# SunJiamei/LRP-ImageCaptioning

Hardware: AMD Instinct MI355X
Metric: LRP heatmaps/sec (per predicted token) VGG16+adaptive-attn, 224x224 (higher is better)
Workload: dtype bf16x3; 1 GPU; batch=32 synthetic 224x224 per GPU, VGG16 + adaptive-attention, LRP per-token heat-maps, 10 words/caption, V=10000 (BASELINE configs[1]); parallelism=image-sharded x1, RCCL weight broadcast, reverse_walk_precision=bf16x3, handles_per_gpu=2

## Files before the change

lrp-imagecaptioning_amd/csrc/conv_args.h:

```cpp
#pragma once

namespace lrp {

enum ConvPrec { PREC_FP32 = 0, PREC_BF16X3 = 1, PREC_F16X2 = 2 };

enum ConvEpi {
  EPI_BIAS_RELU = 0,
  EPI_BIAS = 1,
  EPI_MUL = 2,
  EPI_MUL_UP2 = 3,
  EPI_FWD_DUAL = 4,
  EPI_STORE = 5,
  EPI_IMG_STENCIL = 6
};
constexpr int IMG_PATCH = 16, IMG_TILE = 14;
constexpr int ACT_MAX_SLOTS = 64;

constexpr int LDS_STRIDE = 32;

constexpr int HALO_PITCH = 16, HALO_PL = 4;
constexpr int conv_halo_rows(int BM) { return BM == 256 ? 352 : 192; }

}

// ... 17 lines not shown
    lo[q] = (_Float16)(r[q] - (float)hi[q]);
  }
  u32x4* d = reinterpret_cast<u32x4*>(dst);
  d[0] = __builtin_bit_cast(u32x4, hi);
  d[1] = __builtin_bit_cast(u32x4, lo);
}
__device__ __forceinline__ void split8_store(const float* r, float* dst) {
  bf16x8 hi, lo;
#pragma unroll
  for (int q = 0; q < 8; ++q) {
    hi[q] = (__bf16)r[q];
    lo[q] = (__bf16)(r[q] - (float)hi[q]);
  }
  u32x4* d = reinterpret_cast<u32x4*>(dst);
  d[0] = __builtin_bit_cast(u32x4, hi);
  d[1] = __builtin_bit_cast(u32x4, lo);
}
__device__ __forceinline__ void conv_divmod(int x, int d, float inv, int& q, int& r) {
  q = (int)(((float)x + 0.5f) * inv);
  r = x - q * d;
  if (r < 0) { --q; r += d; } else if (r >= d) { ++q; r -= d; }
}

struct TileOrder {
  std::vector<int> sig;
  int H = 0, th = 0, nyh = 0, cols_t = 0, tpt = 0;
  bool identity = true;
  int* dev = nullptr;
  int* pinned = nullptr;
  size_t cap = 0;
  hipEvent_t ev = nullptr;
  TileOrder() = default;
  TileOrder(const TileOrder&) = delete;
  TileOrder& operator=(const TileOrder&) = delete;
  ~TileOrder() {
    if (dev) (void)hipFree(dev);
    if (pinned) (void)hipHostFree(pinned);
    if (ev) (void)hipEventDestroy(ev);
  }
};

struct ConvArgs {
  const float* in;
  const float* wpk;
  const float* wpk_frag;
  int NB, H, W, Cin, CinP;
  int N;
  int taps;
  int M;
  int m_tiles, n_tiles;
  const float* bias;
  float* out;
  float* out2;
  const float* aux;
// ... 19 lines not shown
  const int* row2img_host;
  const float* tok_fac;
  unsigned* tok_max_out;
  const float* in_unscale;
  unsigned* act_max_out;
  float* pairs_out;
  const float* pairs_scale;
  int skip_out;
  int scale_per_img, img_rows, n_imgs;
  const float* up2_src;
  int gate_none;
  const unsigned char* up2_gpos;
  int up2_pairs;
  const float* img_w;
  float* img_part;
  int tpt;
  int epi_generic;
  float* pool_gc;
  unsigned char* pool_pos;
  float* pool_x;
  const float* aux_b;
  float* out_b;
  int ostride;
};

}
#endif
```

lrp-imagecaptioning_amd/csrc/conv_igemm.h:

```cpp
#pragma once
#include <hip/hip_runtime.h>
#include <stdint.h>

#include "conv_args.h"
#include "conv_plan.h"
#include "conv_tile.h"

namespace lrp {

__device__ __attribute__((aligned(16))) float lrp_zero_page[4] = {0.f, 0.f, 0.f, 0.f};


template <int WM, int WN, int TM, int TN, int EPI, int PREC, bool HALO = false, bool BREG = false, int TERMS = 7, int NS = 2,
          bool GMASK = false, bool PW = false, bool DG = false>
__global__ __launch_bounds__(64 * WM * WN, BREG && WM * WN != 8 && TN == 1 ? 3 : NS > 2 ? 2 : conv_min_waves(WM * WN, TM, TN, HALO)) void conv_igemm_kernel(ConvArgs a) {
#if defined(__HIP_DEVICE_COMPILE__)
  using T = ConvKernelTraits<WM, WN, TM, TN, EPI, PREC, HALO, BREG, TERMS, NS, GMASK, PW, DG>;
  __shared__ __attribute__((aligned(16))) float smem[T::SMEM];

  const int nblk = a.m_tiles * a.n_tiles;
  int logical;
  {
    const int bid = blockIdx.x, q = nblk >> 3, r = nblk & 7, xcd = bid & 7, idx = bid >> 3;
    logical = (xcd < r ? xcd * (q + 1) : r * (q + 1) + (xcd - r) * q) + idx;
  }
  const int mt = logical / a.n_tiles, nt = logical - mt * a.n_tiles;
  const int m0 = mt * T::BM, n0 = nt * T::BN;
  int pn = 0, py0 = 0, px0 = 0;
  if constexpr (EPI == EPI_IMG_STENCIL) {
    const int tpi = a.tiles_x * a.tiles_y;
    pn = mt / tpi;
    const int r = mt - pn * tpi, ty = r / a.tiles_x;
    py0 = ty * IMG_TILE;
    px0 = (r - ty * a.tiles_x) * IMG_TILE;
  }
  int Y0 = 0, x0 = 0, img0 = 0;
  if constexpr (HALO) {
    const int mtp = a.tile_map ? a.tile_map[mt] : mt;
    const int tyt = mtp / a.cols_t;
    x0 = (mtp - tyt * a.cols_t) * a.tw;
    if (a.tpt > 0) {
      img0 = tyt / a.tpt;
      Y0 = img0 * a.H + (tyt - img0 * a.tpt) * a.th;
    } else {
      Y0 = tyt * a.th;
      img0 = Y0 / a.H;
    }
  }
  const int yend = HALO ? (a.tpt > 0 && (img0 + 1) * a.H < a.nyh ? (img0 + 1) * a.H : a.nyh) : 0;
  const float inv_tw = HALO ? 1.0f / (float)a.tw : 0.f, inv_H = HALO ? 1.0f / (float)a.H : 0.f;
  const float inv_H1 = HALO ? 1.0f / (float)(a.H + 1) : 0.f;
  int simg0 = 0;
  float us0 = 1.f, us1 = 1.f, ps0 = 1.f, ps1 = 1.f;
  [[maybe_unused]] const float inv_img_rows = EPI == EPI_FWD_DUAL && a.scale_per_img ? 1.0f / (float)a.img_rows : 0.f;
  if constexpr (EPI == EPI_FWD_DUAL) {
    if (a.dual_il) {
      int simg1 = 0;
      if (a.scale_per_img) {
        simg0 = HALO ? img0 : m0 / a.img_rows;
        simg1 = simg0 + 1 < a.n_imgs ? simg0 + 1 : simg0;
      }
      if constexpr (PREC == PREC_F16X2) { us0 = a.in_unscale[simg0]; us1 = a.in_unscale[simg1]; }
      if (a.pairs_out) { ps0 = a.pairs_scale[simg0]; ps1 = a.pairs_scale[simg1]; }
    }
  }

  const int tid = threadIdx.x, lane = tid & 63, wave = tid >> 6;
  const int wm = wave / WN, wn = wave - wm * WN;
  const int HW = a.H * a.W;
  const int K = a.taps * a.CinP;
  const int cpt = a.CinP >> 5;
  const int nk = a.taps * cpt;

  int prow = lane >> 3, pchk = lane & 7;
  const int wave_s = __builtin_amdgcn_readfirstlane(wave);
  typedef __attribute__((address_space(3))) void* lptr_t;
  constexpr int OOB = (int)0x80000000;
  constexpr int RSRC_FLAGS = 0x00020000;
  const __amdgpu_buffer_rsrc_t rsB =
      __builtin_amdgcn_make_buffer_rsrc((void*)(a.wpk + (size_t)n0 * K), 0, T::BN * K * 4, RSRC_FLAGS);
  int bvo[T::BP];
#pragma unroll
  for (int p = 0; p < T::BP; ++p) {
    const int r = (wave_s * T::BP + p) * 8 + prow;
    bvo[p] = (r * K + ((pchk ^ ((r >> 1) & 7)) << 2)) * 4;
  }
  const float* abase = HALO ? a.in + (size_t)(Y0 > 0 ? Y0 - 1 : 0) * a.W * a.Cin
                       : EPI == EPI_IMG_STENCIL ? a.in + (size_t)pn * HW * a.Cin
                            : a.in + ((long)m0 - (a.taps == 1 ? 0 : a.W + 1)) * (long)a.Cin;
  const __amdgpu_buffer_rsrc_t rsA = __builtin_amdgcn_make_buffer_rsrc((void*)abase, 0, 0x7FFFFFFF, RSRC_FLAGS);
  int avo[HALO ? 1 : T::AP];
// ... 143 lines not shown
  [[maybe_unused]] auto pw_store = [&](const PwItem& w, int it, int chunk, int abuf) {
    if (it >= pw_items) return;
    const PwPos r = pw_locate(it, chunk);
#pragma unroll
    for (int dx = 0; dx < 2; ++dx) {
      const int hx = 2 * r.wx + dx - (x0 - 1);
      if (hx < 0 || hx >= HALO_PITCH) continue;
      const unsigned j = (unsigned)((r.dy << 1) | dx);
      u32x4 mh, ml;
#pragma unroll
      for (int d = 0; d < 4; ++d) {
        const unsigned p0 = (w.q[d >> 1] >> (16 * (d & 1))) & 0xFFu, p1 = (w.q[d >> 1] >> (16 * (d & 1) + 8)) & 0xFFu;
        const unsigned m = r.valid ? ((p0 == j ? 0x0000FFFFu : 0u) | (p1 == j ? 0xFFFF0000u : 0u)) : 0u;
        mh[d] = w.hi[d] & m;
        ml[d] = w.lo[d] & m;
      }
      const int row = r.hy * HALO_PITCH + hx;
      const int swzu = ((r.hy * a.tw + hx - 1) >> 1) & 7;
      const int dst = abuf * T::STAGE + row * LDS_STRIDE + (((2 * r.g) ^ swzu) << 2);
      *reinterpret_cast<u32x4*>(smem + dst) = mh;
      *reinterpret_cast<u32x4*>(smem + (dst ^ 4)) = ml;
    }
  };
  [[maybe_unused]] PwItem pwi{};
  if constexpr (T::BREGC) {
    if constexpr (PW) {
      pw_load(pwi, tid, 0); pw_store(pwi, tid, 0, 0);
      if (tid + T::NT < pw_items) { pw_load(pwi, tid + T::NT, 0); pw_store(pwi, tid + T::NT, 0, 0); }
    } else
    for (int p = wave_s; p < halo_np; p += T::NW) fire_halo_piece(prep_halo_piece(p, 0, true), p, 0);
  } else if constexpr (BREG) {
    if (PREC == PREC_BF16X3 && a.up2_src) {
      const int Hp = a.H >> 1, Wp = a.W >> 1;
      const int h0 = Y0 - img0 * a.H;
      const int wy0 = (h0 - 1) >> 1, wx0 = (x0 - 1) >> 1;
      const int nwx = ((x0 + a.tw) >> 1) - wx0 + 1, nwy = ((h0 + a.th) >> 1) - wy0 + 1;
      const int items = nwy * nwx * 8;
      const int ntok = img0 < a.NB ? img0 : a.NB - 1;
      const int img = a.row2img ? a.row2img[ntok] : ntok;
      const float inv_nwx = 1.0f / (float)nwx;
      constexpr int UW = 2;
      typedef unsigned u32x2_ __attribute__((ext_vector_type(2)));
      for (int it0 = tid; it0 < items; it0 += T::NT * UW) {
        f32x4 pv[UW][2];
        u32x2_ qv[UW];
        int wyv[UW], wxv[UW], cgv[UW];
        bool okv[UW];
#pragma unroll
        for (int u = 0; u < UW; ++u) {
          const int item = it0 + u * T::NT;
          const int cg = item & 7, wdx = item >> 3;
          int wr, wc;
          conv_divmod(wdx, nwx, inv_nwx, wr, wc);
          const int wy = wy0 + wr, wx = wx0 + wc;
// ... 395 lines not shown
      if ((kc & (T::FLUSH - 1)) == T::FLUSH - 1) {
#pragma unroll
        for (int i = 0; i < TM; ++i)
#pragma unroll
          for (int j = 0; j < TN; ++j) {
            tot[i][j] += acc[i][j];
#pragma unroll
            for (int r = 0; r < 16; ++r) acc[i][j][r] = 0.f;
          }
      }
    }
    buf = nbuf;
  }
  conv_dma_landed_barrier();
  if constexpr (T::BLOCKED) {
#pragma unroll
    for (int i = 0; i < TM; ++i)
#pragma unroll
      for (int j = 0; j < TN; ++j) acc[i][j] += tot[i][j];
  }

  if constexpr (BREG && EPI == EPI_MUL && PREC == PREC_BF16X3 && TM == 2 && TN == 1 && WM == 2 && WN == 2) {
    if (a.img_part) {
      static_assert(2 * T::STAGE >= 128 * 64, "the C tile (then S_1 as pairs, in place; then T) inside the staging LDS");
      constexpr int TS2 = 57;
      float* Cs = smem;
      const float inv_tw2 = 1.0f / (float)a.tw;
      f32x4 gq[4][2];
#pragma unroll
      for (int k = 0; k < 4; ++k) {
        const int item = tid + k * T::NT, row = item >> 3, g = item & 7;
        int ty, tx;
        conv_divmod(row, a.tw, inv_tw2, ty, tx);
        const int Y = Y0 + ty, w = x0 + tx;
        const f32x4 z4 = {0.f, 0.f, 0.f, 0.f};
        gq[k][0] = gq[k][1] = z4;
        if (row < a.th * a.tw && Y < yend && w < a.W) {
          int n, h;
          conv_divmod(Y, a.H, inv_H, n, h);
          const int img = a.row2img ? a.row2img[n] : n;
          const float* gp = a.aux + ((size_t)img * HW + h * a.W + w) * a.N + g * 8;
          gq[k][0] = *reinterpret_cast<const f32x4*>(gp); gq[k][1] = *reinterpret_cast<const f32x4*>(gp + 4);
        }
      }
      u32x4 wq[2][2][2][2];
      {
        const int h2 = lane >> 5;
#pragma unroll
        for (int cc = 0; cc < 2; ++cc)
#pragma unroll
          for (int st = 0; st < 2; ++st)
#pragma unroll
            for (int hl = 0; hl < 2; ++hl)
#pragma unroll
              for (int j = 0; j < 2; ++j)
                wq[cc][st][hl][j] = *reinterpret_cast<const u32x4*>(a.img_w + (size_t)(j * 32 + (lane & 31)) * 64 + cc * 32 + (4 * st + 2 * h2 + hl) * 4);
      }
#pragma unroll
      for (int i = 0; i < TM; ++i)
#pragma unroll
        for (int r = 0; r < 16; ++r)
          Cs[((wm * TM + i) * 32 + (r & 3) + 8 * (r >> 2) + 4 * (lane >> 5)) * 64 + wn * 32 + (lane & 31)] = acc[i][0][r];
      __syncthreads();
#pragma unroll
      for (int k = 0; k < 4; ++k) {
        const int item = tid + k * T::NT, row = item >> 3, g = item & 7;
        float* rp = Cs + row * 64 + (g >> 2) * 32;
        const f32x4 c0 = *reinterpret_cast<const f32x4*>(rp + (g & 3) * 8), c1 = *reinterpret_cast<const f32x4*>(rp + (g & 3) * 8 + 4);
        float v[8];
#pragma unroll
        for (int e = 0; e < 4; ++e) { v[e] = c0[e] * gq[k][0][e]; v[4 + e] = c1[e] * gq[k][1][e]; }
        bf16x8 hi, lo;
#pragma unroll
        for (int q = 0; q < 8; ++q) {
          hi[q] = (__bf16)v[q];
          lo[q] = (__bf16)(v[q] - (float)hi[q]);
        }
        const int d = ((2 * (g & 3)) ^ ((row >> 1) & 7)) << 2;
        *reinterpret_cast<u32x4*>(rp + d) = __builtin_bit_cast(u32x4, hi);
        *reinterpret_cast<u32x4*>(rp + (d ^ 4)) = __builtin_bit_cast(u32x4, lo);
      }
      __syncthreads();
      f32x16 t2[2];
#pragma unroll
      for (int j = 0; j < 2; ++j)
#pragma unroll
        for (int r = 0; r < 16; ++r) t2[j][r] = 0.f;
      {
        const int a_row = wave * 32 + (lane & 31), swz2 = (lane >> 1) & 7, h2 = lane >> 5;
#pragma unroll
        for (int cc = 0; cc < 2; ++cc)
#pragma unroll
          for (int st = 0; st < 2; ++st) {
            const bf16x8 ah = __builtin_bit_cast(bf16x8, *reinterpret_cast<const u32x4*>(Cs + a_row * 64 + cc * 32 + (((4 * st + 2 * h2) ^ swz2) << 2)));
            const bf16x8 al = __builtin_bit_cast(bf16x8, *reinterpret_cast<const u32x4*>(Cs + a_row * 64 + cc * 32 + (((4 * st + 2 * h2 + 1) ^ swz2) << 2)));
#pragma unroll
            for (int j = 0; j < 2; ++j) {
              const bf16x8 bh = __builtin_bit_cast(bf16x8, wq[cc][st][0][j]), bl = __builtin_bit_cast(bf16x8, wq[cc][st][1][j]);
              t2[j] = __builtin_amdgcn_mfma_f32_32x32x16_bf16(al, bh, t2[j], 0, 0, 0);
              t2[j] = __builtin_amdgcn_mfma_f32_32x32x16_bf16(ah, bl, t2[j], 0, 0, 0);
              t2[j] = __builtin_amdgcn_mfma_f32_32x32x16_bf16(ah, bh, t2[j], 0, 0, 0);
            }
          }
      }
      __syncthreads();
      float* Ts = smem;
#pragma unroll
      for (int r = 0; r < 16; ++r) {
        const int lr = wave * 32 + (r & 3) + 8 * (r >> 2) + 4 * (lane >> 5);
#pragma unroll
        for (int j = 0; j < 2; ++j) {
          const int col = j * 32 + (lane & 31);
          if (col < TS2) Ts[lr * TS2 + col] = t2[j][r];
        }
      }
      __syncthreads();
      const int RW = a.tw + 2, npos = (a.th + 2) * RW;
      const int mtp_ = a.tile_map ? a.tile_map[mt] : mt;
      for (int p = tid; p < npos; p += T::NT) {
        const int ry = p / RW, rx = p - ry * RW, oy = ry - 1, ox = rx - 1;
        float pos[3] = {0.f, 0.f, 0.f}, neg[3] = {0.f, 0.f, 0.f};
#pragma unroll
        for (int tap = 0; tap < 9; ++tap) {
          const int sy = oy - (tap / 3 - 1), sx = ox - (tap % 3 - 1);
          if (sy >= 0 && sy < a.th && sx >= 0 && sx < a.tw && Y0 + sy < yend && x0 + sx < a.W) {
            const float* r = Ts + (sy * a.tw + sx) * TS2 + tap * 6;
            pos[0] += r[0]; pos[1] += r[1]; pos[2] += r[2];
            neg[0] += r[3]; neg[1] += r[4]; neg[2] += r[5];
          }
        }
        float* o = a.img_part + ((size_t)mtp_ * npos + p) * 6;
        o[0] = pos[0]; o[1] = pos[1]; o[2] = pos[2]; o[3] = neg[0]; o[4] = neg[1]; o[5] = neg[2];
      }
      return;
    }
  }

  if constexpr (EPI == EPI_IMG_STENCIL) {
    constexpr int TS = T::BN + 1;
    static_assert(T::BM == IMG_PATCH * IMG_PATCH && T::BN == 64 && T::BM * TS <= 2 * T::STAGE, "patch tile is 256 x 64");
    float* Ts = smem;
#pragma unroll
    for (int i = 0; i < TM; ++i)
#pragma unroll
      for (int r = 0; r < 16; ++r) {
        const int lr = (wm * TM + i) * 32 + (r & 3) + 8 * (r >> 2) + 4 * (lane >> 5);
#pragma unroll
        for (int j = 0; j < TN; ++j) Ts[lr * TS + (wn * TN + j) * 32 + (lane & 31)] = acc[i][j][r];
      }
    __syncthreads();
    for (int o = tid; o < IMG_TILE * IMG_TILE; o += T::NT) {
      const int oy = o / IMG_TILE, ox = o - oy * IMG_TILE;
      const int y = py0 + oy, x = px0 + ox;
      if (y >= a.H || x >= a.W) continue;
      float pos[3] = {0.f, 0.f, 0.f}, neg[3] = {0.f, 0.f, 0.f};
#pragma unroll
      for (int tap = 0; tap < 9; ++tap) {
        const float* r = Ts + ((oy + 2 - tap / 3) * IMG_PATCH + (ox + 2 - tap % 3)) * TS + tap * 6;
        pos[0] += r[0]; pos[1] += r[1]; pos[2] += r[2];
// ... 585 lines not shown
```

lrp-imagecaptioning_amd/csrc/conv_launch.h:

```cpp
#pragma once
#include <string.h>
#include <algorithm>
#include <utility>
#include <vector>

#include "common.h"
#include "conv_igemm.h"
#include "conv_plan.h"

namespace lrp {

inline const int* conv_tile_order(const ConvArgs& a, hipStream_t st) {
  if (!sw().tile_order || !a.order || !a.row2img_host || a.NB < 2 || a.th < 1) return nullptr;
  TileOrder& o = *a.order;
  const int tiles_y = a.tpt > 0 ? a.NB * a.tpt : (a.nyh + a.th - 1) / a.th;
  const bool same = o.H == a.H && o.th == a.th && o.nyh == a.nyh && o.cols_t == a.cols_t && o.tpt == a.tpt && (int)o.sig.size() == a.NB &&
                    memcmp(o.sig.data(), a.row2img_host, (size_t)a.NB * sizeof(int)) == 0;
  if (same) return o.identity ? nullptr : o.dev;
  o.sig.assign(a.row2img_host, a.row2img_host + a.NB);
  o.H = a.H; o.th = a.th; o.nyh = a.nyh; o.cols_t = a.cols_t; o.tpt = a.tpt;
  constexpr int band = 1, strip = 2;
  std::vector<long long> key((size_t)tiles_y);
  for (int ty = 0; ty < tiles_y; ++ty) {
    int Ym = a.tpt > 0 ? (ty / a.tpt) * a.H + (ty % a.tpt) * a.th + a.th / 2 : ty * a.th + a.th / 2;
    if (a.tpt > 0 && Ym > (ty / a.tpt + 1) * a.H - 1) Ym = (ty / a.tpt + 1) * a.H - 1;
    if (Ym > a.nyh - 1) Ym = a.nyh - 1;
    const int t = Ym / a.H, hpos = Ym - t * a.H;
    key[ty] = ((long long)o.sig[t] << 42) | ((long long)(hpos / (a.th * band)) << 21) | (long long)t;
  }
  std::vector<int> rows((size_t)tiles_y);
  for (int i = 0; i < tiles_y; ++i) rows[i] = i;
// ... 19 lines not shown
    if (o.dev) (void)hipFree(o.dev);
    if (o.pinned) (void)hipHostFree(o.pinned);
    o.dev = o.pinned = nullptr;
    o.cap = 0;
    if (hipMalloc((void**)&o.dev, m_tiles * sizeof(int)) != hipSuccess ||
        hipHostMalloc((void**)&o.pinned, m_tiles * sizeof(int), hipHostMallocDefault) != hipSuccess) {
      (void)hipGetLastError();
      o.sig.clear();
      return nullptr;
    }
    o.cap = m_tiles;
  }
  memcpy(o.pinned, map.data(), m_tiles * sizeof(int));
  if (!o.ev) (void)hipEventCreateWithFlags(&o.ev, hipEventDisableTiming);
  if (hipMemcpyAsync(o.dev, o.pinned, m_tiles * sizeof(int), hipMemcpyHostToDevice, st) != hipSuccess) {
    (void)hipGetLastError();
    o.sig.clear();
    return nullptr;
  }
  (void)hipEventRecord(o.ev, st);
  return o.dev;
}

inline ConvAsk conv_ask(int epi, int prec, int terms, bool gmask, const ConvArgs& a) {
  ConvAsk q;
  q.epi = epi; q.prec = prec; q.terms = terms; q.gmask = gmask;
  q.NB = a.NB; q.H = a.H; q.W = a.W; q.N = a.N; q.Cin = a.Cin; q.taps = a.taps;
  q.frag = a.wpk_frag != nullptr; q.join = a.join != nullptr; q.dual_il = a.dual_il != 0; q.split = a.split;
  q.up2_src = a.up2_src != nullptr; q.img_part = a.img_part != nullptr; q.pool_gc = a.pool_gc != nullptr;
  q.dual_mul = a.out_b != nullptr;
  return q;
}
inline void conv_apply_plan(const ConvPlan& p, ConvArgs& a) {
  a.M = p.M; a.m_tiles = p.m_tiles; a.n_tiles = p.n_tiles;
  a.tw = p.tw; a.th = p.th; a.hrows = p.hrows; a.cols_t = p.cols_t; a.nyh = p.nyh; a.tpt = p.tpt;
  a.epi_generic = p.epi_generic;
}

template <int PREC>
inline hipError_t conv_launch_img(ConvArgs a, hipStream_t st) {
  if (!a.ximg || (PREC == PREC_F16X2 && !a.tok_fac)) return hipErrorInvalidValue;
  const ConvPlan p = conv_plan(conv_ask(EPI_IMG_STENCIL, PREC, 7, false, a));
  if (!p.ok) return hipErrorInvalidValue;
  if (a.NB <= 0) return hipSuccess;
  conv_apply_plan(p, a);
  a.tiles_x = (a.W + IMG_TILE - 1) / IMG_TILE;
  a.tiles_y = (a.H + IMG_TILE - 1) / IMG_TILE;
  hipLaunchKernelGGL((conv_igemm_kernel<4, 1, 2, 2, EPI_IMG_STENCIL, PREC>), dim3(a.m_tiles), dim3(p.threads), 0, st, a);
  return hipGetLastError();
}

template <int I, int EPI, int PREC, int TERMS, bool GMASK, bool DG>
inline bool conv_launch_form(const ConvPlan& p, ConvArgs& a, hipStream_t st) {
  constexpr ConvFormTile F = CONV_FORM_TILES[I];
  if constexpr (conv_kernel_exists(F.form, F.BM, F.BN, F.pw, EPI, PREC, TERMS, GMASK, DG)) {
    if (p.form != F.form || p.BM != F.BM || p.BN != F.BN || p.pw != F.pw) return false;
    constexpr ConvKernelShape K = conv_kernel_shape(F.form, F.BM, F.BN, F.pw);
    if (K.HALO && (EPI == EPI_MUL || EPI == EPI_MUL_UP2)) a.tile_map = conv_tile_order(a, st);
    hipLaunchKernelGGL((conv_igemm_kernel<K.WM, K.WN, K.TM, K.TN, EPI, PREC, K.HALO, K.BREG, TERMS, K.NS, GMASK, K.PW, DG>),
                       dim3(p.m_tiles * p.n_tiles), dim3(p.threads), 0, st, a);
    return true;
  }
  return false;
}
template <int EPI, int PREC, int TERMS, bool GMASK, bool DG, int... I>
inline bool conv_launch_forms(const ConvPlan& p, ConvArgs& a, hipStream_t st, std::integer_sequence<int, I...>) {
  return (conv_launch_form<I, EPI, PREC, TERMS, GMASK, DG>(p, a, st) || ...);
}

template <int EPI, int PREC, int TERMS = 7, bool GMASK = false, bool DG = false>
inline hipError_t conv_launch_epi(ConvArgs a, hipStream_t st) {
  static_assert(EPI != EPI_IMG_STENCIL && conv_epi_exists(EPI, PREC, TERMS, GMASK, DG), "conv_plan.h: no kernel has this epilogue in this format");
  constexpr bool MUL = EPI == EPI_MUL || EPI == EPI_MUL_UP2, FWD = EPI == EPI_BIAS || EPI == EPI_BIAS_RELU || EPI == EPI_FWD_DUAL;
  if (DG != (a.out_b != nullptr)) return hipErrorInvalidValue;
  if (DG && (!a.aux || !a.aux_b || !a.out || a.ostride < a.N || (a.ostride & (PREC != PREC_FP32 ? 7 : 3)) || a.out2s || a.gate_none ||
             a.gate_binary || a.relu_out))
    return hipErrorInvalidValue;
  if (GMASK && (a.out2s || a.gate_none)) return hipErrorInvalidValue;
  if (PREC == PREC_F16X2 && MUL && (!a.tok_fac || !a.tok_max_out || a.out_plain)) return hipErrorInvalidValue;
  if (PREC == PREC_F16X2 && FWD && !a.in_unscale) return hipErrorInvalidValue;
// ... 40 lines not shown
```

lrp-imagecaptioning_amd/csrc/conv_plan.h:

```cpp
#pragma once
#include "conv_args.h"
#include "switches.h"

namespace lrp {

struct ConvTile { int BM, BN; };
inline ConvTile conv_pick_tile(int N) {
  if (N > 64) return {128, 128};
  if (N > 32) return {128, 64};
  return {128, 32};
}
inline int conv_npad(int N) { ConvTile t = conv_pick_tile(N); return (N + t.BN - 1) / t.BN * t.BN; }
inline int conv_cinp(int Cin) { return (Cin + 31) / 32 * 32; }

enum ConvForm {
  FORM_PLAIN = 0,
  FORM_SMALL = 1,
  FORM_HALO = 2,
  FORM_BREG = 3,
  FORM_POOL = 4,
  FORM_IMG = 5,
  FORM_BREG8 = 6,
  FORM_BREG4 = 7,
  FORM_BREG4_POOL = 8
// ... 63 lines not shown
struct ConvKernelShape { int WM, WN, TM, TN; bool HALO, BREG; int NS; bool PW; };
constexpr ConvKernelShape conv_kernel_shape(int form, int BM, int BN, bool pw) {
  const bool breg = form == FORM_BREG || form == FORM_BREG8 || form == FORM_BREG4 || form == FORM_BREG4_POOL;
  const bool halo = breg || form == FORM_HALO || form == FORM_POOL;
  const int ns = form == FORM_SMALL ? CONV_SMALL_NS : 2;
  if (form == FORM_IMG) return {4, 1, 2, 2, false, false, 2, false};
  if (BM == 256) return {2, 4, 4, 2, halo, breg, ns, pw};
  if (BM == 64) return {2, 2, 1, 1, halo, breg, ns, pw};
  if (BN == 128) return {2, 2, 2, 2, halo, breg, ns, pw};
  if (BN == 64) return {2, 2, 2, 1, halo, breg, ns, pw};
  return {4, 1, 1, 1, halo, breg, ns, pw};
}
constexpr bool conv_kernel_instantiated(int WM, int WN, int TM, int TN, bool HALO, bool BREG, int NS, bool PW, int epi, int prec, int terms,
                                        bool gmask, bool dual) {
  for (const ConvFormTile& f : CONV_FORM_TILES) {
    const ConvKernelShape k = conv_kernel_shape(f.form, f.BM, f.BN, f.pw);
    if (k.WM == WM && k.WN == WN && k.TM == TM && k.TN == TN && k.HALO == HALO && k.BREG == BREG && k.NS == NS && k.PW == PW &&
        conv_kernel_exists(f.form, f.BM, f.BN, f.pw, epi, prec, terms, gmask, dual))
      return true;
  }
  return false;
}

inline float conv_halo_geom(int BM, int H, int W, bool even, int& tw, int& th, int& hrows) {
  const int avail = conv_halo_rows(BM) / HALO_PITCH;
  const int step = even ? 2 : 1;
  float best = 0.f;
  for (int c = step; c <= HALO_PITCH - 2 && c <= W; c += step) {
    int t = even ? (BM / c) & ~1 : BM / c;
    while (t > 0 && t + 2 + (t - 1 + H - 1) / H > avail) t -= step;
    if (t < step) continue;
    const int cols = (W + c - 1) / c;
    const float u = (float)(t * c) / (float)BM * (float)W / (float)(cols * c);
    if (u > best + 1e-6f) { best = u; tw = c; th = t; hrows = t + 2 + (t - 1 + H - 1) / H; }
  }
  return best;
}

inline bool conv_compact_shape(int N, int Cin, int H, int W) {
  if ((Cin & 7) || (H & 1) || (W & 1)) return false;
  return conv_pick_tile(N).BN == 128  || (N <= 64 && conv_cinp(Cin) <= 64) ;
}

inline unsigned conv_frag_forms(int epi, int prec, int terms, int N, int Cin, int taps, const Switches& s = sw()) {
  if (taps != 9 || N <= 0 || (Cin & 7)) return 0;
  auto has = [&](int form, int BM, int BN) { return conv_kernel_exists(form, BM, BN, false, epi, prec, terms, false, false); };
// ... 105 lines not shown
```

lrp-imagecaptioning_amd/csrc/conv_tile.h:

```cpp
#pragma once
#include <hip/hip_runtime.h>
#include <stdint.h>

#include "conv_args.h"
#include "conv_plan.h"

namespace lrp {

constexpr int conv_min_waves(int NW, int TM, int TN, bool halo = false) { return NW == 8 || halo ? 2 : (TM * TN >= 4 ? 2 : 3); }

template <int WM_, int WN_, int TM_, int TN_, int EPI_, int PREC_, bool HALO_, bool BREG_, int TERMS_, int NS_, bool GMASK_, bool PW_, bool DG_>
struct ConvKernelTraits {
  static constexpr int WM = WM_, WN = WN_, TM = TM_, TN = TN_, EPI = EPI_, PREC = PREC_, TERMS = TERMS_, NS = NS_;
  static constexpr bool HALO = HALO_, BREG = BREG_, GMASK = GMASK_, PW = PW_, DG = DG_;

  static constexpr int NW = WM * WN, NT = 64 * NW;
  static constexpr bool SPLIT = PREC != PREC_FP32;
  static constexpr int BM = WM * TM * 32, BN = WN * TN * 32;
  static constexpr int AP = BM / 8 / NW, BP = BN / 8 / NW;
  static constexpr int HR = conv_halo_rows(BM);
  static constexpr int ABUF = (HALO ? HR : BM) * LDS_STRIDE;
  static constexpr int STAGE = ABUF + (BREG ? 0 : BN) * LDS_STRIDE;
  static constexpr bool BREG8 = BREG && NW == 8;
  static constexpr bool BREG4 = BREG && NW == 4 && TN == 2;
// ... 11 lines not shown
  static constexpr int CSLAB = BREGC ? SMEM : 2 * STAGE;

  static constexpr int NSTEP = SPLIT ? 2 : 4;
  static_assert(!BREG || NSTEP == 2, "weights in registers: split operands");
  static_assert(!BREGC || SMEM >= 2 * STAGE + NW * 8 * LDS_STRIDE, "a spare LDS slot per wave behind the two images");
  static_assert(!BREGC || 6 * NW * 8 >= HR, "six piece slots per wave cover the resident image");
  static constexpr int FLUSH = 8;
  static constexpr bool BLOCKED = PREC == PREC_FP32 || (PREC == PREC_F16X2 && (EPI == EPI_BIAS || EPI == EPI_BIAS_RELU || EPI == EPI_FWD_DUAL));

  static constexpr bool SLABS = EPI != EPI_STORE && EPI != EPI_IMG_STENCIL;
  static constexpr int NH = (BM * BN + CSLAB - 1) / CSLAB;
  static constexpr int RH = BM / NH;
  static_assert(!SLABS || (BM % NH == 0 && RH % (TM * 32) == 0 && RH * BN <= CSLAB), "slab must hold whole wave tiles");
  static constexpr bool SPLIT_OUT = SPLIT && (EPI == EPI_MUL || EPI == EPI_MUL_UP2);
  static constexpr int CW = SPLIT_OUT ? 8 : 4;
  static constexpr int C4 = BN / CW, RPP = NT / C4;
  static constexpr bool TMAX_LDS = PREC == PREC_F16X2 && RH * BN + 16 <= 2 * STAGE;
};

__device__ __forceinline__ void conv_dma_landed_barrier() {
  asm volatile("s_waitcnt vmcnt(0)" ::: "memory");
  __syncthreads();
}
template <class T>
__device__ __forceinline__ void conv_dma_oldest_landed_barrier() {
  if constexpr (T::NS > 2) {
    asm volatile("s_waitcnt vmcnt(%0)" ::"n"((T::NS - 2) * T::DPC) : "memory");
    __syncthreads();
  } else {
    conv_dma_landed_barrier();
  }
}

}
```

lrp-imagecaptioning_amd/csrc/switches.h:

```cpp
#pragma once
#include <cstdlib>

namespace lrp {

struct Switches {
  int conv_halo = 1;
  int conv_breg = 1;
  int conv_breg8 = 1;
  int conv_breg4 = 1;
  int conv_sparse_wreg = 1;
  int conv_small = 1;
  int conv_mid = 1;
  int epi_fast = 1;
  int up2_pw = 1;
  int tile_order = 1;
  int fwd_emit = 1;
  int fwd_il = 1;
  int img_fused = 1;
  int up2_compact = 1;
  int img_fold = 1;
  int pool_fused = 1;
  int sparse_pool = 1;
  void load() {
    *this = Switches();
    auto rd = [](const char* name, int& v) { if (const char* e = getenv(name)) v = atoi(e); };
    rd("LRP_CONV_HALO", conv_halo); rd("LRP_CONV_BREG", conv_breg); rd("LRP_CONV_SMALL", conv_small);
    rd("LRP_CONV_MID", conv_mid); rd("LRP_EPI_FAST", epi_fast); rd("LRP_UP2_PW", up2_pw); rd("LRP_TILE_ORDER", tile_order);
    rd("LRP_FWD_EMIT", fwd_emit); rd("LRP_FWD_IL", fwd_il); rd("LRP_IMG_FUSED", img_fused); rd("LRP_UP2_COMPACT", up2_compact);
    rd("LRP_IMG_FOLD", img_fold); rd("LRP_SPARSE_POOL", sparse_pool); rd("LRP_POOL_FUSED", pool_fused);
    if (const char* e = getenv("LRP_CONV_BREG8")) conv_breg8 = atoi(e);
    if (const char* e = getenv("LRP_CONV_BREG4")) conv_breg4 = atoi(e);
    if (const char* e = getenv("LRP_CONV_SPARSE_WREG")) conv_sparse_wreg = atoi(e);
  }
};
inline Switches& sw() {
  static Switches s = [] { Switches t; t.load(); return t; }();
  return s;
}

}
```

Baseline: 11200 heatmaps/s.

## Process runs of same-image tokens per block in the BREG image-part conv

Adds a run-table path for the BF16x3 EPI_MUL image-part kernel. Each block now loops over several tokens that share an image and tile position, so the block setup, weight registers and gate loads are reused across tokens. The next token's up2 source data is prefetched during the current token's epilogue. A host-built, cached run table sets the grid size, and the run length is chosen so the grid still fills the CUs. The cost is fewer blocks, a serial per-block loop, and extra register pressure and code complexity.

```diff
diff --git a/lrp-imagecaptioning_amd/csrc/conv_args.h b/lrp-imagecaptioning_amd/csrc/conv_args.h
--- a/lrp-imagecaptioning_amd/csrc/conv_args.h
+++ b/lrp-imagecaptioning_amd/csrc/conv_args.h
@@ -63,6 +63,23 @@
   if (r < 0) { --q; r += d; } else if (r >= d) { ++q; r -= d; }
 }
 
+struct RunCache {
+  std::vector<int> sig;
+  int tpt = 0, cols_t = 0, cap = 0;
+  int n_runs = 0, n_toks = 0;
+  int* dev = nullptr;
+  int* pinned = nullptr;
+  size_t size = 0;
+  hipEvent_t ev = nullptr;
+  RunCache() = default;
+  RunCache(const RunCache&) = delete;
+  RunCache& operator=(const RunCache&) = delete;
+  ~RunCache() {
+    if (dev) (void)hipFree(dev);
+    if (pinned) (void)hipHostFree(pinned);
+    if (ev) (void)hipEventDestroy(ev);
+  }
+};
 struct TileOrder {
   std::vector<int> sig;
   int H = 0, th = 0, nyh = 0, cols_t = 0, tpt = 0;
@@ -71,6 +88,7 @@
   int* pinned = nullptr;
   size_t cap = 0;
   hipEvent_t ev = nullptr;
+  RunCache runs;
   TileOrder() = default;
   TileOrder(const TileOrder&) = delete;
   TileOrder& operator=(const TileOrder&) = delete;
@@ -136,6 +154,9 @@
   const float* aux_b;
   float* out_b;
   int ostride;
+  const int* run_tab;
+  const int* run_toks;
+  int n_runs;
 };
 
 }
diff --git a/lrp-imagecaptioning_amd/csrc/conv_igemm.h b/lrp-imagecaptioning_amd/csrc/conv_igemm.h
--- a/lrp-imagecaptioning_amd/csrc/conv_igemm.h
+++ b/lrp-imagecaptioning_amd/csrc/conv_igemm.h
@@ -12,13 +12,14 @@
 
 
 template <int WM, int WN, int TM, int TN, int EPI, int PREC, bool HALO = false, bool BREG = false, int TERMS = 7, int NS = 2,
-          bool GMASK = false, bool PW = false, bool DG = false>
+          bool GMASK = false, bool PW = false, bool DG = false, bool RUN = false>
 __global__ __launch_bounds__(64 * WM * WN, BREG && WM * WN != 8 && TN == 1 ? 3 : NS > 2 ? 2 : conv_min_waves(WM * WN, TM, TN, HALO)) void conv_igemm_kernel(ConvArgs a) {
 #if defined(__HIP_DEVICE_COMPILE__)
   using T = ConvKernelTraits<WM, WN, TM, TN, EPI, PREC, HALO, BREG, TERMS, NS, GMASK, PW, DG>;
+  static_assert(!RUN || conv_run_kernel_exists(WM, WN, TM, TN, HALO, BREG, NS, PW, EPI, PREC, TERMS, GMASK, DG), "no such run instantiation: conv_plan.h");
   __shared__ __attribute__((aligned(16))) float smem[T::SMEM];
 
-  const int nblk = a.m_tiles * a.n_tiles;
+  const int nblk = RUN ? a.n_runs : a.m_tiles * a.n_tiles;
   int logical;
   {
     const int bid = blockIdx.x, q = nblk >> 3, r = nblk & 7, xcd = bid & 7, idx = bid >> 3;
@@ -35,8 +36,15 @@
     px0 = (r - ty * a.tiles_x) * IMG_TILE;
   }
   int Y0 = 0, x0 = 0, img0 = 0;
+  [[maybe_unused]] int run_place = 0, run_n = 1, run_first = 0, run_img = 0, cur_tok = 0, nxt_tok = 0, rk = 0;
   if constexpr (HALO) {
-    const int mtp = a.tile_map ? a.tile_map[mt] : mt;
+    int mtp;
+    if constexpr (RUN) {
+      const int4 rd = reinterpret_cast<const int4*>(a.run_tab)[mt];
+      run_place = rd.x & 0xFFFFFF; run_n = rd.x >> 24; run_first = rd.y; run_img = rd.z; cur_tok = rd.w;
+      mtp = cur_tok * (a.tpt * a.cols_t) + run_place;
+    } else
+    mtp = a.tile_map ? a.tile_map[mt] : mt;
     const int tyt = mtp / a.cols_t;
     x0 = (mtp - tyt * a.cols_t) * a.tw;
     if (a.tpt > 0) {
@@ -65,8 +73,8 @@
     }
   }
 
-  const int tid = threadIdx.x, lane = tid & 63, wave = tid >> 6;
-  const int wm = wave / WN, wn = wave - wm * WN;
+  int tid = threadIdx.x, lane = tid & 63, wave = tid >> 6;
+  int wm = wave / WN, wn = wave - wm * WN;
   const int HW = a.H * a.W;
   const int K = a.taps * a.CinP;
   const int cpt = a.CinP >> 5;
@@ -256,6 +264,85 @@
       *reinterpret_cast<u32x4*>(smem + (dst ^ 4)) = ml;
     }
   };
+  constexpr int UWR = 2;
+  typedef unsigned u32x2r __attribute__((ext_vector_type(2)));
+  struct Up2Geom { int Hp, Wp, h0, wy0, wx0, nwx, items; float inv_nwx; };
+  struct Up2Items { f32x4 pv[UWR][2]; u32x2r qv[UWR]; };
+  [[maybe_unused]] auto up2_geom = [&]() {
+    Up2Geom G;
+    G.Hp = a.H >> 1; G.Wp = a.W >> 1;
+    G.h0 = Y0 - img0 * a.H;
+    G.wy0 = (G.h0 - 1) >> 1; G.wx0 = (x0 - 1) >> 1;
+    G.nwx = ((x0 + a.tw) >> 1) - G.wx0 + 1;
+    const int nwy = ((G.h0 + a.th) >> 1) - G.wy0 + 1;
+    G.items = nwy * G.nwx * 8;
+    G.inv_nwx = 1.0f / (float)G.nwx;
+    return G;
+  };
+  [[maybe_unused]] auto up2_item = [&](const Up2Geom& G, int item, int& cg, int& wy, int& wx) {
+    cg = item & 7;
+    int wr, wc;
+    conv_divmod(item >> 3, G.nwx, G.inv_nwx, wr, wc);
+    wy = G.wy0 + wr; wx = G.wx0 + wc;
+    return item < G.items && wy >= 0 && wy < G.Hp && wx >= 0 && wx < G.Wp && cg * 8 < a.Cin;
+  };
+  [[maybe_unused]] auto up2_load = [&](const Up2Geom& G, int it0, int ntok, int img, Up2Items& w) {
+#pragma unroll
+    for (int u = 0; u < UWR; ++u) {
+      int cg, wy, wx;
+      (void)up2_item(G, it0 + u * T::NT, cg, wy, wx);
+      const int wyc = wy < 0 ? 0 : (wy >= G.Hp ? G.Hp - 1 : wy), wxc = wx < 0 ? 0 : (wx >= G.Wp ? G.Wp - 1 : wx);
+      const int cgc = cg * 8 < a.Cin ? cg : 0;
+      const size_t wo = ((size_t)wyc * G.Wp + wxc) * a.Cin + cgc * 8;
+      const float* pp = a.up2_src + (size_t)ntok * G.Hp * G.Wp * a.Cin + wo;
+      w.pv[u][0] = *reinterpret_cast<const f32x4*>(pp); w.pv[u][1] = *reinterpret_cast<const f32x4*>(pp + 4);
+      w.qv[u] = *reinterpret_cast<const u32x2r*>(a.up2_gpos + (size_t)img * G.Hp * G.Wp * a.Cin + wo);
+    }
+  };
+  [[maybe_unused]] auto up2_build = [&](const Up2Geom& G, int it0, const Up2Items& w) {
+#pragma unroll
+    for (int u = 0; u < UWR; ++u) {
+      if (it0 + u * T::NT >= G.items) continue;
+      int cg, wy, wx;
+      const bool ok = up2_item(G, it0 + u * T::NT, cg, wy, wx);
+      const u32x4 z4u = {0u, 0u, 0u, 0u};
+      const u32x4 hiw = ok ? __builtin_bit_cast(u32x4, w.pv[u][0]) : z4u;
+      const u32x4 low = ok ? __builtin_bit_cast(u32x4, w.pv[u][1]) : z4u;
+#pragma unroll
+      for (int j = 0; j < 4; ++j) {
+        const int hy = 2 * wy + (j >> 1) - (G.h0 - 1), hx = 2 * wx + (j & 1) - (x0 - 1);
+        if (hy < 0 || hy >= a.hrows || hx < 0 || hx >= HALO_PITCH) continue;
+        u32x4 mh, ml;
+#pragma unroll
+        for (int d = 0; d < 4; ++d) {
+          const unsigned p0 = (w.qv[u][d >> 1] >> (16 * (d & 1))) & 0xFFu, p1 = (w.qv[u][d >> 1] >> (16 * (d & 1) + 8)) & 0xFFu;
+          const unsigned m = (p0 == (unsigned)j ? 0x0000FFFFu : 0u) | (p1 == (unsigned)j ? 0xFFFF0000u : 0u);
+          mh[d] = hiw[d] & m;
+          ml[d] = low[d] & m;
+        }
+        const int row = hy * HALO_PITCH + hx;
+        const int swzu = ((hy * a.tw + hx - 1) >> 1) & 7;
+        const int dst = (cg >> 2) * T::STAGE + row * LDS_STRIDE + (((2 * (cg & 3)) ^ swzu) << 2);
+        *reinterpret_cast<u32x4*>(smem + dst) = mh;
+        *reinterpret_cast<u32x4*>(smem + (dst ^ 4)) = ml;
+      }
+    }
+  };
+  [[maybe_unused]] Up2Items up2w;
+  if constexpr (RUN) {
+    up2_load(up2_geom(), tid, cur_tok, run_img, up2w);
+    up2_build(up2_geom(), tid, up2w);
+  }
+  do {
+  if constexpr (RUN) {
+    asm volatile("" : "+v"(tid), "+s"(Y0), "+s"(x0), "+s"(img0));
+    lane = tid & 63; wave = tid >> 6;
+    wm = wave / WN; wn = wave - wm * WN;
+#pragma unroll
+    for (int i = 0; i < TM; ++i)
+#pragma unroll
+      for (int r = 0; r < 16; ++r) acc[i][0][r] = 0.f;
+  }
   [[maybe_unused]] PwItem pwi{};
   if constexpr (T::BREGC) {
     if constexpr (PW) {
@@ -264,6 +351,9 @@
     } else
     for (int p = wave_s; p < halo_np; p += T::NW) fire_halo_piece(prep_halo_piece(p, 0, true), p, 0);
   } else if constexpr (BREG) {
+    if constexpr (RUN) {
+      nxt_tok = rk + 1 < run_n ? a.run_toks[run_first + rk + 1] : cur_tok;
+    } else
     if (PREC == PREC_BF16X3 && a.up2_src) {
       const int Hp = a.H >> 1, Wp = a.W >> 1;
       const int h0 = Y0 - img0 * a.H;
@@ -705,11 +795,29 @@
 
   if constexpr (BREG && EPI == EPI_MUL && PREC == PREC_BF16X3 && TM == 2 && TN == 1 && WM == 2 && WN == 2) {
     if (a.img_part) {
+      auto epi_barrier = [] {
+        if constexpr (RUN) conv_lds_barrier();
+        else __syncthreads();
+      };
       static_assert(2 * T::STAGE >= 128 * 64, "the C tile (then S_1 as pairs, in place; then T) inside the staging LDS");
       constexpr int TS2 = 57;
       float* Cs = smem;
       const float inv_tw2 = 1.0f / (float)a.tw;
       f32x4 gq[4][2];
+      [[maybe_unused]] bool okg[4] = {true, true, true, true};
+      if constexpr (RUN) {
+#pragma unroll
+        for (int k = 0; k < 4; ++k) {
+          const int item = tid + k * T::NT, row = item >> 3, g = item & 7;
+          int ty = (int)(((float)row + 0.5f) * inv_tw2), tx = row - ty * a.tw;
+          const int up = tx < 0 ? -1 : tx >= a.tw ? 1 : 0;
+          ty += up; tx -= up * a.tw;
+          const int h = Y0 - img0 * a.H + ty, w = x0 + tx;
+          okg[k] = row < a.th * a.tw && h < a.H && w < a.W;
+          const float* gp = a.aux + ((size_t)run_img * HW + (okg[k] ? h * a.W + w : (Y0 - img0 * a.H) * a.W + x0)) * a.N + g * 8;
+          gq[k][0] = *reinterpret_cast<const f32x4*>(gp); gq[k][1] = *reinterpret_cast<const f32x4*>(gp + 4);
+        }
+      } else
 #pragma unroll
       for (int k = 0; k < 4; ++k) {
         const int item = tid + k * T::NT, row = item >> 3, g = item & 7;
@@ -744,13 +852,17 @@
 #pragma unroll
         for (int r = 0; r < 16; ++r)
           Cs[((wm * TM + i) * 32 + (r & 3) + 8 * (r >> 2) + 4 * (lane >> 5)) * 64 + wn * 32 + (lane & 31)] = acc[i][0][r];
-      __syncthreads();
+      epi_barrier();
 #pragma unroll
       for (int k = 0; k < 4; ++k) {
         const int item = tid + k * T::NT, row = item >> 3, g = item & 7;
         float* rp = Cs + row * 64 + (g >> 2) * 32;
         const f32x4 c0 = *reinterpret_cast<const f32x4*>(rp + (g & 3) * 8), c1 = *reinterpret_cast<const f32x4*>(rp + (g & 3) * 8 + 4);
         float v[8];
+        if constexpr (RUN) {
+          const f32x4 z4 = {0.f, 0.f, 0.f, 0.f};
+          if (!okg[k]) gq[k][0] = gq[k][1] = z4;
+        }
 #pragma unroll
         for (int e = 0; e < 4; ++e) { v[e] = c0[e] * gq[k][0][e]; v[4 + e] = c1[e] * gq[k][1][e]; }
         bf16x8 hi, lo;
@@ -763,7 +875,7 @@
         *reinterpret_cast<u32x4*>(rp + d) = __builtin_bit_cast(u32x4, hi);
         *reinterpret_cast<u32x4*>(rp + (d ^ 4)) = __builtin_bit_cast(u32x4, lo);
       }
-      __syncthreads();
+      epi_barrier();
       f32x16 t2[2];
 #pragma unroll
       for (int j = 0; j < 2; ++j)
@@ -786,7 +898,11 @@
             }
           }
       }
-      __syncthreads();
+      epi_barrier();
+      if constexpr (RUN) {
+        if (rk + 1 < run_n) up2_load(up2_geom(), tid, nxt_tok, run_img, up2w);
+        else up2w = Up2Items{};
+      }
       float* Ts = smem;
 #pragma unroll
       for (int r = 0; r < 16; ++r) {
@@ -797,9 +913,11 @@
           if (col < TS2) Ts[lr * TS2 + col] = t2[j][r];
         }
       }
-      __syncthreads();
+      epi_barrier();
       const int RW = a.tw + 2, npos = (a.th + 2) * RW;
-      const int mtp_ = a.tile_map ? a.tile_map[mt] : mt;
+      int mtp_;
+      if constexpr (RUN) mtp_ = cur_tok * (a.tpt * a.cols_t) + run_place;
+      else mtp_ = a.tile_map ? a.tile_map[mt] : mt;
       for (int p = tid; p < npos; p += T::NT) {
         const int ry = p / RW, rx = p - ry * RW, oy = ry - 1, ox = rx - 1;
         float pos[3] = {0.f, 0.f, 0.f}, neg[3] = {0.f, 0.f, 0.f};
@@ -815,9 +933,18 @@
         float* o = a.img_part + ((size_t)mtp_ * npos + p) * 6;
         o[0] = pos[0]; o[1] = pos[1]; o[2] = pos[2]; o[3] = neg[0]; o[4] = neg[1]; o[5] = neg[2];
       }
+      if constexpr (RUN) {
+        if (++rk < run_n) {
+          cur_tok = nxt_tok;
+          epi_barrier();
+          up2_build(up2_geom(), tid, up2w);
+          continue;
+        }
+      }
       return;
     }
   }
+  } while (RUN);
 
   if constexpr (EPI == EPI_IMG_STENCIL) {
     constexpr int TS = T::BN + 1;
diff --git a/lrp-imagecaptioning_amd/csrc/conv_launch.h b/lrp-imagecaptioning_amd/csrc/conv_launch.h
--- a/lrp-imagecaptioning_amd/csrc/conv_launch.h
+++ b/lrp-imagecaptioning_amd/csrc/conv_launch.h
@@ -7,6 +7,7 @@
 #include "common.h"
 #include "conv_igemm.h"
 #include "conv_plan.h"
+#include "conv_runs.h"
 
 namespace lrp {
 
@@ -72,6 +73,63 @@
   return o.dev;
 }
 
+inline bool conv_run_table(ConvArgs& a, hipStream_t st) {
+  const Switches& s = sw();
+  if (!s.conv_breg_run || s.conv_breg_run_max == 1 || !a.order || !a.row2img_host || !a.row2img || !a.img_part || !a.up2_src ||
+      a.tpt < 1 || a.NB < 2 || a.n_tiles != 1 || a.CinP > 64)
+    return false;
+  if (((a.th + 1) / 2 + 2) * ((a.tw + 1) / 2 + 2) * 8 > 2 * 256) return false;
+  if ((long long)a.NB * a.tpt * a.cols_t > 0x7FFFFFFFLL) return false;
+  RunCache& c = a.order->runs;
+  const bool same = c.tpt == a.tpt && c.cols_t == a.cols_t && c.cap == s.conv_breg_run_max && (int)c.sig.size() == a.NB &&
+                    memcmp(c.sig.data(), a.row2img_host, (size_t)a.NB * sizeof(int)) == 0;
+  if (!same) {
+    c.sig.assign(a.row2img_host, a.row2img_host + a.NB);
+    c.tpt = a.tpt; c.cols_t = a.cols_t; c.cap = s.conv_breg_run_max;
+    c.n_runs = 0;
+    static const int cus = [] {
+      int dev = 0, n = 0;
+      if (hipGetDevice(&dev) != hipSuccess || hipDeviceGetAttribute(&n, hipDeviceAttributeMultiprocessorCount, dev) != hipSuccess) (void)hipGetLastError();
+      return n > 0 ? n : 256;
+    }();
+    const int cap = conv_run_cap(c.sig.data(), a.NB, a.tpt * a.cols_t, cus, s.conv_breg_run_max);
+    if (cap > 1) {
+      ConvRunTable t;
+      conv_build_runs(c.sig.data(), a.NB, a.tpt, a.cols_t, cap, t);
+      const size_t need = t.runs.size() + t.toks.size();
+      if (c.ev) (void)hipEventSynchronize(c.ev);
+      if (c.size < need) {
+        if (c.dev) (void)hipFree(c.dev);
+        if (c.pinned) (void)hipHostFree(c.pinned);
+        c.dev = c.pinned = nullptr;
+        c.size = 0;
+        if (hipMalloc((void**)&c.dev, need * sizeof(int)) != hipSuccess ||
+            hipHostMalloc((void**)&c.pinned, need * sizeof(int), hipHostMallocDefault) != hipSuccess) {
+          (void)hipGetLastError();
+          c.sig.clear();
+          return false;
+        }
+        c.size = need;
+      }
+      if (t.n_runs() > 0) {
+        memcpy(c.pinned, t.runs.data(), t.runs.size() * sizeof(int));
+        memcpy(c.pinned + t.runs.size(), t.toks.data(), t.toks.size() * sizeof(int));
+        if (!c.ev) (void)hipEventCreateWithFlags(&c.ev, hipEventDisableTiming);
+        if (hipMemcpyAsync(c.dev, c.pinned, need * sizeof(int), hipMemcpyHostToDevice, st) != hipSuccess) {
+          (void)hipGetLastError();
+          c.sig.clear();
+          return false;
+        }
+        (void)hipEventRecord(c.ev, st);
+        c.n_runs = t.n_runs(); c.n_toks = (int)t.toks.size();
+      }
+    }
+  }
+  if (c.n_runs < 1) return false;
+  a.run_tab = c.dev; a.run_toks = c.dev + (size_t)c.n_runs * 4; a.n_runs = c.n_runs;
+  return true;
+}
+
 inline ConvAsk conv_ask(int epi, int prec, int terms, bool gmask, const ConvArgs& a) {
   ConvAsk q;
   q.epi = epi; q.prec = prec; q.terms = terms; q.gmask = gmask;
@@ -106,6 +164,13 @@
   if constexpr (conv_kernel_exists(F.form, F.BM, F.BN, F.pw, EPI, PREC, TERMS, GMASK, DG)) {
     if (p.form != F.form || p.BM != F.BM || p.BN != F.BN || p.pw != F.pw) return false;
     constexpr ConvKernelShape K = conv_kernel_shape(F.form, F.BM, F.BN, F.pw);
+    if constexpr (conv_run_kernel_exists(F.form, F.BM, F.BN, F.pw, EPI, PREC, TERMS, GMASK, DG)) {
+      if (conv_run_table(a, st)) {
+        hipLaunchKernelGGL((conv_igemm_kernel<K.WM, K.WN, K.TM, K.TN, EPI, PREC, K.HALO, K.BREG, TERMS, K.NS, GMASK, K.PW, DG, true>),
+                           dim3(a.n_runs), dim3(p.threads), 0, st, a);
+        return true;
+      }
+    }
     if (K.HALO && (EPI == EPI_MUL || EPI == EPI_MUL_UP2)) a.tile_map = conv_tile_order(a, st);
     hipLaunchKernelGGL((conv_igemm_kernel<K.WM, K.WN, K.TM, K.TN, EPI, PREC, K.HALO, K.BREG, TERMS, K.NS, GMASK, K.PW, DG>),
                        dim3(p.m_tiles * p.n_tiles), dim3(p.threads), 0, st, a);
diff --git a/lrp-imagecaptioning_amd/csrc/conv_plan.h b/lrp-imagecaptioning_amd/csrc/conv_plan.h
--- a/lrp-imagecaptioning_amd/csrc/conv_plan.h
+++ b/lrp-imagecaptioning_amd/csrc/conv_plan.h
@@ -109,6 +109,17 @@
   return false;
 }
 
+constexpr bool conv_run_kernel_exists(int form, int BM, int BN, bool pw, int epi, int prec, int terms, bool gmask, bool dual) {
+  return form == FORM_BREG && BM == 128 && BN == 64 && !pw && epi == EPI_MUL && prec == PREC_BF16X3 && !gmask && !dual &&
+         conv_kernel_exists(form, BM, BN, pw, epi, prec, terms, gmask, dual);
+}
+constexpr bool conv_run_kernel_exists(int WM, int WN, int TM, int TN, bool HALO, bool BREG, int NS, bool PW, int epi, int prec, int terms,
+                                      bool gmask, bool dual) {
+  const ConvKernelShape k = conv_kernel_shape(FORM_BREG, 128, 64, false);
+  return k.WM == WM && k.WN == WN && k.TM == TM && k.TN == TN && k.HALO == HALO && k.BREG == BREG && k.NS == NS && k.PW == PW &&
+         conv_run_kernel_exists(FORM_BREG, 128, 64, false, epi, prec, terms, gmask, dual);
+}
+
 inline float conv_halo_geom(int BM, int H, int W, bool even, int& tw, int& th, int& hrows) {
   const int avail = conv_halo_rows(BM) / HALO_PITCH;
   const int step = even ? 2 : 1;
diff --git a/lrp-imagecaptioning_amd/csrc/conv_runs.h b/lrp-imagecaptioning_amd/csrc/conv_runs.h
--- /dev/null
+++ b/lrp-imagecaptioning_amd/csrc/conv_runs.h
@@ -0,0 +1,66 @@
+#pragma once
+#include <algorithm>
+#include <vector>
+
+namespace lrp {
+
+struct ConvRunTable {
+  std::vector<int> toks;
+  std::vector<int> runs;
+  int n_runs() const { return (int)(runs.size() / 4); }
+};
+constexpr int CONV_RUN_MAX = 127;
+constexpr int CONV_RUN_MAX_PLACES = 1 << 24;
+
+inline long conv_run_count(const int* tok2img, int n_tok, int places, int cap) {
+  std::vector<int> img(tok2img, tok2img + n_tok);
+  std::sort(img.begin(), img.end());
+  long runs = 0;
+  for (int i = 0; i < n_tok;) {
+    int j = i;
+    while (j < n_tok && img[j] == img[i]) ++j;
+    runs += (j - i + cap - 1) / cap;
+    i = j;
+  }
+  return runs * places;
+}
+inline int conv_run_cap(const int* tok2img, int n_tok, int places, int cus, int want) {
+  if (n_tok < 1 || places < 1) return 1;
+  if (want > 0) return want < CONV_RUN_MAX ? want : CONV_RUN_MAX;
+  std::vector<int> img(tok2img, tok2img + n_tok);
+  std::sort(img.begin(), img.end());
+  int longest = 1;
+  for (int i = 0, j = 0; i < n_tok; i = j) {
+    while (j < n_tok && img[j] == img[i]) ++j;
+    longest = std::max(longest, j - i);
+  }
+  int cap = std::min(longest, CONV_RUN_MAX);
+  const long fill = 4L * 3 * cus;
+  while (cap > 1 && conv_run_count(tok2img, n_tok, places, cap) < fill) cap = (cap + 1) / 2;
+  return cap;
+}
+
+inline void conv_build_runs(const int* tok2img, int n_tok, int tpt, int cols_t, int cap, ConvRunTable& t) {
+  t.toks.resize((size_t)(n_tok > 0 ? n_tok : 0));
+  t.runs.clear();
+  if (n_tok < 1 || tpt < 1 || cols_t < 1 || (long)tpt * cols_t > CONV_RUN_MAX_PLACES) return;
+  cap = cap < 1 ? 1 : cap > CONV_RUN_MAX ? CONV_RUN_MAX : cap;
+  for (int i = 0; i < n_tok; ++i) t.toks[i] = i;
+  std::stable_sort(t.toks.begin(), t.toks.end(), [&](int x, int y) { return tok2img[x] < tok2img[y]; });
+  constexpr int strip = 2;
+  for (int i0 = 0; i0 < n_tok;) {
+    int i1 = i0;
+    while (i1 < n_tok && tok2img[t.toks[i1]] == tok2img[t.toks[i0]]) ++i1;
+    for (int c0 = 0; c0 < cols_t; c0 += strip)
+      for (int r = 0; r < tpt; ++r)
+        for (int c = c0; c < c0 + strip && c < cols_t; ++c)
+          for (int f = i0; f < i1; f += cap) {
+            const int cnt = std::min(cap, i1 - f);
+            const int rec[4] = {(r * cols_t + c) | (cnt << 24), f, tok2img[t.toks[i0]], t.toks[f]};
+            t.runs.insert(t.runs.end(), rec, rec + 4);
+          }
+    i0 = i1;
+  }
+}
+
+}
diff --git a/lrp-imagecaptioning_amd/csrc/conv_tile.h b/lrp-imagecaptioning_amd/csrc/conv_tile.h
--- a/lrp-imagecaptioning_amd/csrc/conv_tile.h
+++ b/lrp-imagecaptioning_amd/csrc/conv_tile.h
@@ -57,6 +57,7 @@
   asm volatile("s_waitcnt vmcnt(0)" ::: "memory");
   __syncthreads();
 }
+__device__ __forceinline__ void conv_lds_barrier() { asm volatile("s_waitcnt lgkmcnt(0)\n\ts_barrier" ::: "memory"); }
 template <class T>
 __device__ __forceinline__ void conv_dma_oldest_landed_barrier() {
   if constexpr (T::NS > 2) {
diff --git a/lrp-imagecaptioning_amd/csrc/switches.h b/lrp-imagecaptioning_amd/csrc/switches.h
--- a/lrp-imagecaptioning_amd/csrc/switches.h
+++ b/lrp-imagecaptioning_amd/csrc/switches.h
@@ -21,6 +21,8 @@
   int img_fold = 1;
   int pool_fused = 1;
   int sparse_pool = 1;
+  int conv_breg_run = 1;
+  int conv_breg_run_max = 0;
   void load() {
     *this = Switches();
     auto rd = [](const char* name, int& v) { if (const char* e = getenv(name)) v = atoi(e); };
@@ -31,6 +33,8 @@
     if (const char* e = getenv("LRP_CONV_BREG8")) conv_breg8 = atoi(e);
     if (const char* e = getenv("LRP_CONV_BREG4")) conv_breg4 = atoi(e);
     if (const char* e = getenv("LRP_CONV_SPARSE_WREG")) conv_sparse_wreg = atoi(e);
+    if (const char* e = getenv("LRP_CONV_BREG_RUN")) conv_breg_run = atoi(e);
+    if (const char* e = getenv("LRP_CONV_BREG_RUN_MAX")) conv_breg_run_max = atoi(e);
   }
 };
 inline Switches& sw() {
diff --git a/profiles/breg_run_ab.py b/profiles/breg_run_ab.py
--- /dev/null
+++ b/profiles/breg_run_ab.py
@@ -0,0 +1,58 @@
+#!/usr/bin/env python3
+import os, sys, statistics
+import numpy as np
+sys.path.insert(0, os.path.dirname(os.path.dirname(os.path.abspath(__file__))))
+PASSES = int(sys.argv[1]) if len(sys.argv) > 1 else 5
+CAPS = [int(a) for a in sys.argv[2:]] or [0, 5, 2]
+import torch
+from bench import synth_weights
+from lrp_imagecaptioning_amd.engine import LRPEngine, switches
+from lrp_imagecaptioning_amd.synthetic import VGG16_CFG, captions, images
+B, T, V = 32, 10, 10000
+eng = LRPEngine(decoder="adaptive", V=V, max_images=B, max_tokens=B * T, max_caption_len=T + 1)
+eng.set_weights(synth_weights(0, V))
+rs = np.random.RandomState(1)
+X = torch.as_tensor(images(rs, B)).cuda()
+caps = captions(rs, B, T, V)
+idx = [b for b in range(B) for _ in range(T)]
+tpos = [t for _ in range(B) for t in range(1, T + 1)]
+out = torch.empty((B * T, 224, 224, 3), dtype=torch.float32, device="cuda")
+eng.encode_images(X); eng.decoder_forward(caps)
+names = [c[0] for c in VGG16_CFG][::-1]
+
+
+def line(name, v0, v1):
+    won = statistics.median(v1) < min(v0)
+    print("%-14s %28s %28s %s" % (name, "%.3f [%.3f, %.3f]" % (statistics.median(v0), min(v0), max(v0)),
+                                  "%.3f [%.3f, %.3f]" % (statistics.median(v1), min(v1), max(v1)), "WON" if won else ""))
+
+
+for cap in CAPS:
+    print("==== LRP_CONV_BREG_RUN_MAX=%d" % cap, flush=True)
+    ref = {}
+    for on in (1, 0):
+        with switches(LRP_CONV_BREG_RUN=on, LRP_CONV_BREG_RUN_MAX=cap):
+            eng.explain_tokens(idx, tpos, out=out); torch.cuda.synchronize()
+            ref[on] = out.clone()
+    print("heat-maps bit-identical on/off:", bool(torch.equal(ref[0], ref[1])), "finite:", bool(torch.isfinite(ref[1]).all()),
+          "non-zero:", float(ref[1].abs().sum()) > 0, flush=True)
+    del ref
+    res = {0: [], 1: []}
+    for p in range(PASSES):
+        for on in (0, 1):
+            with switches(LRP_CONV_BREG_RUN=on, LRP_CONV_BREG_RUN_MAX=cap):
+                eng.explain_tokens(idx, tpos, out=out); torch.cuda.synchronize()
+                eng.profile_enable(True)
+                acc = None
+                for _ in range(3):
+                    eng.explain_tokens(idx, tpos, out=out); torch.cuda.synchronize()
+                    rec = eng.profile_records()
+                    acc = rec if acc is None else [(a + b, f) for (a, f), (b, _) in zip(acc, rec)]
+                eng.profile_enable(False)
+                res[on].append([m / 3 for m, _ in acc])
+            print("pass %d RUN=%d walk %.3f ms: %s" % (p, on, sum(res[on][-1]), " ".join("%.3f" % m for m in res[on][-1])), flush=True)
+    print("records per walk:", len(res[0][0]), names[:len(res[0][0])])
+    print("%-14s %28s %28s" % ("launch", "RUN=0 med [min,max]", "RUN=1 med [min,max]"))
+    for k in range(len(res[0][0])):
+        line(names[k] if k < len(names) else str(k), [r[k] for r in res[0]], [r[k] for r in res[1]])
+    line("walk total", [sum(r) for r in res[0]], [sum(r) for r in res[1]])
```

Result: no change. 11270 heatmaps/s, median of 6 (+0.7%).
